# arneschneuing/DiffSBDD

Hardware: AMD Instinct MI355X
Metric: sampled ligands/sec (500-step DDPM, fullatom_cond) at 1/2/4/8 MI355X (higher is better)
Workload: dtype f32

## Files before the change

diffsbdd_amd/_lib.py:

```python
from __future__ import annotations

import ctypes as C
import os

_HERE = os.path.dirname(os.path.abspath(__file__))
LIB_PATH = os.environ.get("DSBDD_LIB") or os.path.join(_HERE, "libdiffsbdd_hip.so")
ABI_VERSION = 6

OK, ERR_ARG, ERR_STATE, ERR_CAPACITY, ERR_LAUNCH = 0, -1, -2, -3, -4
STATUS_NAN, STATUS_EDGE_OVERFLOW = 1, 2
MOL_MAX_ATOMS, MOL_STATS, FP_WORDS = 128, 8, 64

G_NAMES = ["ATOM_ENC_W0T", "ATOM_ENC_B0", "ATOM_ENC_W1T", "ATOM_ENC_B1",
           "RES_ENC_W0T", "RES_ENC_B0", "RES_ENC_W1T", "RES_ENC_B1",
           "ATOM_DEC_W0T", "ATOM_DEC_B0", "ATOM_DEC_W1T", "ATOM_DEC_B1",
           "RES_DEC_W0T", "RES_DEC_B0", "RES_DEC_W1T", "RES_DEC_B1",
           "EMB_WT", "EMB_B", "EMBOUT_WT", "EMBOUT_B"]
GCL_NAMES = ["E1_WT", "E1_WD", "E1_WD0", "E1_TAB", "E2_WT", "E2_B", "ATT_W", "ATT_B",
             "N1_WT", "N1_B", "N2_WT", "N2_B"]
EQ_NAMES = ["C1_WT", "C_WD", "C_WD0", "C_TAB", "C_W2T", "C_B2",
            "X_WD", "X_WD0", "X_TAB", "X_W2T", "X_B2", "W3"]
OPT_PRUNE, OPT_CONE, OPT_GRANULE16, OPT_EMU, OPT_SPLITK, OPT_SHELL, OPT_TAIL = 0, 1, 2, 3, 4, 5, 6
(BUF_EDGE_ROW, BUF_EDGE_COL, BUF_EDGE_D0, BUF_ROW_PTR, BUF_H, BUF_X, BUF_NODE_BATCH, BUF_DEG,
 BUF_LEVEL, BUF_LEVEL_LIST, BUF_LEVEL_COUNT, BUF_LEVEL_END, BUF_LROW_PTR, BUF_LEDGE_ROW, BUF_LEDGE_COL,
# ... 32 lines not shown
                ("gd0", C.c_void_p)]


class OptimCfg(C.Structure):
    _fields_ = [(n, C.c_double) for n in ("lr", "beta1", "beta2", "eps", "weight_decay")] + [("clip_grad", C.c_int32)]


_P = C.c_void_p
_I64 = C.c_int64
_I32 = C.c_int32
_F = C.c_float

SIGNATURES = {
    "dsbdd_abi_version": (C.c_int, []),
    "dsbdd_last_error": (C.c_char_p, []),
    "dsbdd_engine_create": (C.c_int, [C.POINTER(Config), C.POINTER(_P)]),
    "dsbdd_engine_destroy": (None, [_P]),
    "dsbdd_engine_weight_slots": (C.c_int, [_P]),
    "dsbdd_engine_set_weights": (C.c_int, [_P, C.POINTER(_P), C.c_int]),
    "dsbdd_engine_workspace_bytes": (C.c_size_t, [_P, _I64, _I64, _I64, _I64]),
    "dsbdd_engine_bind_workspace": (C.c_int, [_P, _P, C.c_size_t, _I64, _I64, _I64, _I64]),
    "dsbdd_engine_set_trace": (C.c_int, [_P, _P, _P]),
    "dsbdd_engine_set_pocket_frame": (C.c_int, [_P, _P, _P, _P, _P, _P, _I64, _I64, _I64, _I64, _I64, _I64]),
    "dsbdd_engine_clear_pocket_frame": (C.c_int, [_P]),
    "dsbdd_dynamics_forward": (C.c_int, [_P, _P, _P, _P, _P, _I64, _P, _P, _I64, _I64, _I64,
                                         _P, _P, _I64, _P, _P, _P]),
    "dsbdd_engine_buffer": (C.c_int, [_P, C.c_int, C.POINTER(_P)]),
    "dsbdd_engine_shell_read": (C.c_int, [_P, C.c_int, C.c_int, _P, C.c_int64]),
    "dsbdd_engine_list2_read": (C.c_int, [_P, C.c_int, _P, C.c_int64]),
    "dsbdd_engine_graph_stats": (C.c_int, [_P, C.POINTER(_I64), C.POINTER(_I64), C.POINTER(_I64)]),
    "dsbdd_engine_last_plan": (C.c_int, [_P, C.POINTER(C.c_int32), C.POINTER(C.c_int32), C.c_int32,
                                         C.POINTER(C.c_int32), C.POINTER(C.c_int32)]),
    "dsbdd_engine_set_option": (C.c_int, [_P, C.c_int, C.c_int]),
    "dsbdd_engine_get_option": (C.c_int, [_P, C.c_int]),
    "dsbdd_engine_profile": (C.c_int, [_P, C.c_int, C.c_int]),
    "dsbdd_engine_profile_read": (C.c_int, [_P, C.POINTER(C.c_double), C.POINTER(_I64)]),
    "dsbdd_cond_reverse_update": (C.c_int, [_P, _P, _P, _P, _P, _P, _P, _I64, _I64, _I64,
                                            _I32, _I32, _F, _F, _F, _I32]),
    "dsbdd_joint_reverse_update": (C.c_int, [_P, _P, _P, _P, _P, _P, _P, _P, _P, _I64, _I64, _I64,
                                             _I32, _I32, _F, _F, _F, _I32]),
    "dsbdd_segment_mean3": (C.c_int, [_P, _P, _I32, _P, _I64, _I64, _P]),
    "dsbdd_cond_affine_noise": (C.c_int, [_P, _P, _P, _P, _P, _P, _I64, _I64, _I64, _I32, _I32, _F, _F, _I32]),
    "dsbdd_joint_affine_noise": (C.c_int, [_P, _P, _P, _P, _P, _P, _P, _I64, _I64, _I64, _I32, _I32, _F, _F,
                                           _I32, _I32]),
    "dsbdd_cond_repaint_update": (C.c_int, [_P, _P, _P, _P, _P, _P, _P, _P, _P, _P, _P, _I64, _I64, _I64,
                                            _I32, _I32, _F, _F, _F, _F, _I32, _I32]),
    "dsbdd_joint_repaint_update": (C.c_int, [_P] * 15 + [_I64, _I64, _I64, _I32, _I32, _F, _F, _F, _F, _I32]),
    "dsbdd_cond_step_keyed": (C.c_int, [_P] * 10 + [_I64, _I64, _I64, _I32, _I32, _F, _F, _F, _I32, _F, _F, _F, _I32,
                                        C.c_uint64, C.c_uint64, _I64, _P, _P, _F]),
    "dsbdd_randn_keyed": (C.c_int, [_P, _P, _P, _I64, _I32, _I64, _I64, _P, C.c_uint64, C.c_uint64,
                                    C.c_uint32]),
    "dsbdd_node_linear": (C.c_int, [_P, _P, _I32, _I32, _P, _I32, _I32, _P, _I32, _P, _P, _I32,
                                    _P, _I32, _I64, _I32, _I32]),
    "dsbdd_chain_split_host": (_I64, [_I32, _I32, _I32, _P, _P, _P, _I32, _I32, _P, _P, _I64]),
    "dsbdd_chain_split_probe": (C.c_int, [_P, _I32, _P, _I32, _I32, _P, _P, _P, _I32, _I32, _P, _P, _I64, _P]),
    "dsbdd_build_edges": (C.c_int, [_P, _P, _P, _P, _I64, _I64, _I64, C.POINTER(Config),
                                    _P, _P, _P, _P, _P, _P, _P, _P, _I64, _P]),
    "dsbdd_bond_orders": (C.c_int, [_P, _P, _P, _P, _I64, _I32, _P, _P, _P, C.c_float, C.c_float,
                                    C.c_float, _I32, _P]),
    "dsbdd_mol_graph_stats": (C.c_int, [_P, _P, _P, _P, _I64, _I32, _P, _I32, _I32, _P, _P, _P, _P, _P, _P]),
    "dsbdd_fp_diversity": (C.c_int, [_P, _P, _P, _I64, _P, _P]),
    "dsbdd_pose_check": (C.c_int, [_P, _P, _P, _P, _I64, _P, _P, _P, _P, _I64, _F, _F, _P, _P]),
    "dsbdd_vina_type": (C.c_int, [_P, _P, _P, _P, _I64, _I32, _P, _I32, _P, _P]),
    "dsbdd_vina_score": (C.c_int, [_P, _P, _P, _P, _I64, _P, _P, _P, _P, _P, _I64, _P, _P, _P]),
    "dsbdd_pack_ligands": (C.c_int, [_P, _P, _P, _P, _I32, _I64, _P, _P, _P, _I64, _I64, _I32, _P, _P, _P, _P, _P]),
    "dsbdd_train_scratch_bytes": (C.c_size_t, [_I32, _I64, _I64]),
    "dsbdd_train_wgrad_scratch_bytes": (C.c_size_t, [_I64, _I64, _I64]),
    "dsbdd_train_wgrad_plan_bytes": (C.c_size_t, [_I64, _I64, _I64]),
    "dsbdd_train_edge_rev": (C.c_int, [_P, _P, _P]),
    "dsbdd_train_sample_mean": (C.c_int, [_P, _P, _P, _P]),
    "dsbdd_train_gcl_forward": (C.c_int, [_P, _I32, _P, _P, _P, _F, _P, _P, C.c_size_t]),
    "dsbdd_train_gcl_backward": (C.c_int, [_P, _I32, _P, _P, _P, _F, _P, _P, _P, _P, C.c_size_t]),
    "dsbdd_train_coord_forward": (C.c_int, [_P, _I32, _P, _P, _I32, _P, _P, _I64, _F, _F, _I32, _F, _P, _P,
                                            C.c_size_t]),
    "dsbdd_train_coord_backward": (C.c_int, [_P, _I32, _P, _P, _I32, _P, _P, _I64, _I64, _F, _F, _I32, _F, _P, _P, _P,
                                             _P, _P, C.c_size_t]),
    "dsbdd_train_radial_backward": (C.c_int, [_P, _P, _P, _P, _P]),
    "dsbdd_train_wgrad": (C.c_int, [_P, _P, _I32, _P, _I32, _I64, _I32, _I32, _P, _P, C.c_size_t]),
    "dsbdd_train_colsum": (C.c_int, [_P, _P, _I32, _I64, _I32, _P, _P, C.c_size_t]),
    "dsbdd_train_net_create": (C.c_int, [C.POINTER(Config), C.POINTER(_P)]),
    "dsbdd_train_net_destroy": (None, [_P]),
    "dsbdd_train_net_param_count": (C.c_int, [_P]),
    "dsbdd_train_net_pack_bytes": (C.c_size_t, [_P]),
    "dsbdd_train_net_workspace_bytes": (C.c_size_t, [_P, C.POINTER(TrainGraph)]),
    "dsbdd_train_net_forward": (C.c_int, [_P, _P, C.POINTER(TrainGraph), C.POINTER(_P), _P, C.c_size_t, _P, C.c_size_t, _P, _P,
                                          _P, _I64, _I32, _P, _P, _P]),
    "dsbdd_train_net_backward": (C.c_int, [_P, _P, C.POINTER(TrainGraph), C.POINTER(_P), C.POINTER(_P), _P, C.c_size_t, _P,
                                           C.c_size_t, _I64, _P, _P, _P, _P]),
    "dsbdd_train_net_forward_held": (C.c_int, [_P, _P, C.POINTER(TrainGraph), C.POINTER(_P), _P, C.c_size_t, _P, C.c_size_t,
                                               _P, _P, _P, _I64, _I32, _P, _P, _P, _I32]),
    "dsbdd_train_net_backward_acc": (C.c_int, [_P, _P, C.POINTER(TrainGraph), C.POINTER(_P), C.POINTER(_P), _P, _P, C.c_size_t,
                                               _P, C.c_size_t, _I64, _P, _P, _P, _P]),
    "dsbdd_edge_capacity": (C.c_int, [_P, _P, _I64, _P, _I64, _I64, _P]),
    "dsbdd_loss_rows": (C.c_int, []),
    "dsbdd_loss_out_rows": (C.c_int, []),
    "dsbdd_loss_cond_pre": (C.c_int, [_P, C.POINTER(LossCfg)] + [_P] * 17),
    "dsbdd_loss_cond_post": (C.c_int, [_P, C.POINTER(LossCfg)] + [_P] * 8),
    "dsbdd_loss_cond_post_backward": (C.c_int, [_P, C.POINTER(LossCfg)] + [_P] * 9),
    "dsbdd_loss_joint_out_rows": (C.c_int, []),
    "dsbdd_loss_joint_pre": (C.c_int, [_P, C.POINTER(LossCfg)] + [_P] * 20),
    "dsbdd_loss_joint_post": (C.c_int, [_P, C.POINTER(LossCfg)] + [_P] * 10),
    "dsbdd_loss_joint_post_backward": (C.c_int, [_P, C.POINTER(LossCfg)] + [_P] * 14),
    "dsbdd_score_rows": (C.c_int, [_I32]),
    "dsbdd_score_cond_pre": (C.c_int, [_P, C.POINTER(LossCfg), _I32, _I64, _I64, _I64, _I64] + [_P] * 17),
    "dsbdd_score_cond_post": (C.c_int, [_P, C.POINTER(LossCfg), _I32, _I64, _I64, _I64, _I64] + [_P] * 7),
    "dsbdd_score_reduce": (C.c_int, [_P, _I64, _I32, _P, _P, _P, _P]),
# ... 60 lines not shown
```

diffsbdd_amd/csrc/capi_kernels.h:

```cpp
#pragma once

extern "C" {

int dsbdd_cond_reverse_update(void* stream, float* z_lig, float* xh_pocket, const float* eps_lig,
                              const float* noise, const int64_t* mask_lig, const int64_t* mask_pocket,
                              int64_t n_lig, int64_t n_pocket, int64_t batch, int32_t atom_nf,
                              int32_t residue_nf, float alpha_ts, float c_eps, float sigma, int32_t remove_com) {
  StreamDevice stream_device_(stream);
  if (!z_lig || !xh_pocket || !eps_lig || !noise || !mask_lig || !mask_pocket || batch < 1)
    return fail(DSBDD_ERR_ARG, "bad argument");
  hipLaunchKernelGGL(cond_update_kernel, dim3((int)batch), dim3(kThreads), 0, static_cast<hipStream_t>(stream),
                     z_lig, xh_pocket, eps_lig, noise, mask_lig, (int)n_lig, mask_pocket, (int)n_pocket,
                     3 + atom_nf, 3 + residue_nf, alpha_ts, c_eps, sigma, remove_com);
  HIP_TRY(hipGetLastError());
  return DSBDD_OK;
}

int dsbdd_joint_reverse_update(void* stream, float* z_lig, float* z_pocket, const float* eps_lig,
                               const float* eps_pocket, const float* noise_lig, const float* noise_pocket,
                               const int64_t* mask_lig, const int64_t* mask_pocket, int64_t n_lig,
                               int64_t n_pocket, int64_t batch, int32_t atom_nf, int32_t residue_nf,
                               float alpha_ts, float c_eps, float sigma, int32_t center_noise) {
  StreamDevice stream_device_(stream);
  if (!z_lig || !z_pocket || !eps_lig || !eps_pocket || !noise_lig || !noise_pocket || !mask_lig ||
// ... 81 lines not shown
  a.eps = eps_lig; a.u_alpha_ts = alpha_ts; a.u_c_eps = c_eps; a.u_sigma = sigma; a.repaint = repaint;
  a.seed = seed; a.draw = draw_index; a.sample_offset = sample_offset; a.sample_ids = sample_ids;
  a.t_word = t_word; a.t_next = t_next;
  hipLaunchKernelGGL(cond_step_keyed_kernel, dim3((int)batch), dim3(kThreads), 0, static_cast<hipStream_t>(stream), a);
  HIP_TRY(hipGetLastError());
  return DSBDD_OK;
}

int dsbdd_joint_repaint_update(void* stream, float* z_lig, float* z_pocket, float* scratch_lig,
                               float* scratch_pocket, const float* xh0_lig, const float* xh0_pocket,
                               const float* fixed_lig, const float* fixed_pocket, const float* noise_known_lig,
                               const float* noise_known_pocket, const float* noise_jump_lig,
                               const float* noise_jump_pocket, const int64_t* mask_lig,
                               const int64_t* mask_pocket, int64_t n_lig, int64_t n_pocket, int64_t batch,
                               int32_t atom_nf, int32_t residue_nf, float alpha_s, float sigma_s,
                               float alpha_ts, float sigma_ts, int32_t jump) {
  StreamDevice stream_device_(stream);
  if (!z_lig || !z_pocket || !scratch_lig || !scratch_pocket || !xh0_lig || !xh0_pocket || !fixed_lig ||
      !fixed_pocket || !noise_known_lig || !noise_known_pocket || (jump && (!noise_jump_lig || !noise_jump_pocket)) ||
      !mask_lig || !mask_pocket || batch < 1)
    return fail(DSBDD_ERR_ARG, "bad argument");
  JointRepaintArgs a{z_lig, z_pocket, scratch_lig, scratch_pocket, xh0_lig, xh0_pocket, fixed_lig, fixed_pocket,
                     noise_known_lig, noise_known_pocket, noise_jump_lig, noise_jump_pocket, mask_lig, mask_pocket,
                     (int)n_lig, (int)n_pocket, 3 + atom_nf, 3 + residue_nf, alpha_s, sigma_s, alpha_ts, sigma_ts,
                     jump};
  hipLaunchKernelGGL(joint_repaint_kernel, dim3((int)batch), dim3(kThreads), 0, static_cast<hipStream_t>(stream), a);
  HIP_TRY(hipGetLastError());
  return DSBDD_OK;
}

int dsbdd_randn_keyed(void* stream, float* out, const int64_t* mask, int64_t n_rows, int32_t n_cols,
                      int64_t batch, int64_t sample_offset, const int64_t* sample_ids, uint64_t seed,
                      uint64_t draw_index, uint32_t stream_id) {
  StreamDevice stream_device_(stream);
  (void)batch;
  if (!out || !mask || n_rows < 0 || n_cols < 1) return fail(DSBDD_ERR_ARG, "bad argument");
  const int64_t n = n_rows * n_cols;
  if (n == 0) return DSBDD_OK;
  hipLaunchKernelGGL(randn_keyed_kernel, dim3((int)((n + 255) / 256)), dim3(256), 0,
                     static_cast<hipStream_t>(stream), out, mask, (int)n_rows, (int)n_cols, sample_offset,
                     sample_ids, seed, draw_index, stream_id);
  HIP_TRY(hipGetLastError());
  return DSBDD_OK;
}

int dsbdd_node_linear(void* stream, const float* A1, int32_t lda1, int32_t K1, const float* A2, int32_t lda2,
                      int32_t K2, const float* WT, int32_t ldw, const float* bias, const float* R, int32_t ldr,
                      float* C, int32_t ldc, int64_t M, int32_t N, int32_t act) {
  StreamDevice stream_device_(stream);
  if (!A1 || !WT || !C || K1 < 1 || K2 < 0 || (K2 > 0 && !A2) || (ldw & 3) || N > ldw ||
      (reinterpret_cast<uintptr_t>(WT) & 15))
    return fail(DSBDD_ERR_ARG, "bad argument (WT must be 16-byte aligned with ldw % 4 == 0)");
  HIP_TRY(nl(static_cast<hipStream_t>(stream), A1, lda1, K1, A2, lda2, K2, WT, ldw, bias, R, ldr, C, ldc, M, N, act));
  return DSBDD_OK;
}

static bool chain_split_args_ok(int32_t M, int32_t n_proj, const void* proj_N, const void* proj_first, const void* proj_count,
                                int32_t H, int32_t grid, const void* header, const void* pieces, int64_t capacity) {
  return header && capacity >= 0 && (capacity == 0 || pieces) && grid >= 1 && (H == 64 || H == 128 || H == 192 || H == 256) &&
         n_proj >= 0 && n_proj <= kChainMaxProj && (n_proj == 0 || (proj_N && proj_first && proj_count)) && M <= (8 << 20);
}
static const char* const kChainSplitBadArg =
    "bad argument (null output, grid < 1, H not 64 / 128 / 192 / 256, more than 3 projections or more than 8 M rows)";

int64_t dsbdd_chain_split_host(int32_t M, int32_t do_mlp, int32_t n_proj, const int32_t* proj_N,
                               const int32_t* proj_first, const int32_t* proj_count, int32_t H, int32_t grid,
                               uint32_t* header, int32_t* pieces, int64_t capacity) {
  if (!chain_split_args_ok(M, n_proj, proj_N, proj_first, proj_count, H, grid, header, pieces, capacity))
    return fail(DSBDD_ERR_ARG, kChainSplitBadArg);
  ChainSplitIn in{};
  in.M = M; in.do_mlp = do_mlp; in.n_proj = n_proj; in.H = H; in.grid = grid;
  for (int q = 0; q < n_proj; ++q) { in.N[q] = proj_N[q]; in.first[q] = proj_first[q]; in.count[q] = proj_count[q]; }
  const ChainSplit sp(in);
  sp.report(header);
  return chain_split_list(sp, grid, grid, ~0u, pieces, capacity);
}

int dsbdd_chain_split_probe(void* stream, int32_t M, const int32_t* m_count, int32_t do_mlp, int32_t n_proj,
                            const int32_t* proj_N, const int32_t* proj_first, const int32_t* const* proj_count,
                            int32_t H, int32_t grid, uint32_t* header, int32_t* pieces, int64_t capacity,
                            int64_t* n_pieces) {
  StreamDevice stream_device_(stream);
  if (!n_pieces || !chain_split_args_ok(M, n_proj, proj_N, proj_first, proj_count, H, grid, header, pieces, capacity))
    return fail(DSBDD_ERR_ARG, kChainSplitBadArg);
  NodeChainArgs a{};
  a.M = M; a.m_count = m_count; a.do_mlp = do_mlp; a.n_proj = n_proj;
  for (int q = 0; q < n_proj; ++q) { a.proj[q].N = proj_N[q]; a.proj[q].first = proj_first[q]; a.proj[q].count = proj_count[q]; }
  hipLaunchKernelGGL(chain_split_probe_kernel, dim3(grid), dim3(64), 0, static_cast<hipStream_t>(stream), a, (int)H, header,
                     pieces, (long long)capacity, reinterpret_cast<long long*>(n_pieces));
  HIP_TRY(hipGetLastError());
  return DSBDD_OK;
}

int dsbdd_bond_orders(void* stream, const float* x, const int32_t* atom_type, const int32_t* mol_off,
                      int64_t batch, int32_t n_types, const float* bonds1, const float* bonds2,
                      const float* bonds3, float margin1, float margin2, float margin3, int32_t n_max,
                      int8_t* order) {
  StreamDevice stream_device_(stream);
  if (!x || !atom_type || !mol_off || !bonds1 || !bonds2 || !bonds3 || !order || batch < 1 || n_types < 1 ||
      n_max < 1)
    return fail(DSBDD_ERR_ARG, "bad argument");
  hipStream_t s = static_cast<hipStream_t>(stream);
  HIP_TRY(hipMemsetAsync(order, 0, (size_t)batch * n_max * n_max, s));
  BondArgs a{x, atom_type, mol_off, bonds1, bonds2, bonds3, margin1, margin2, margin3, n_types, n_max,
             reinterpret_cast<signed char*>(order)};
  hipLaunchKernelGGL(bond_orders_kernel, dim3((unsigned)batch), dim3(64), 0, s, a);
// ... 132 lines not shown
```

diffsbdd_amd/csrc/geometry.h:

```cpp
#pragma once
#include "common.h"
#include "graph_parts.h"
#include "radius_graph.h"

namespace dsbdd {

__global__ void prep_assemble_kernel(const int64_t* mask_lig, int n_lig, const int64_t* mask_poc, int n_poc, int B,
                                     int* node_batch, int* lig_off, int* poc_off, int* tile_ctr, const float* xh_lig,
                                     int dl, const float* xh_poc, int dp, const float* t, int t_count, float* x,
                                     float* x_in, float* h0, int J, int JP) {
  const int i = blockIdx.x * blockDim.x + threadIdx.x;
  prep_offsets(i, mask_lig, n_lig, mask_poc, n_poc, B, lig_off, poc_off, tile_ctr);
  if (i >= n_lig + n_poc) return;
  const int b = prep_node(i, mask_lig, n_lig, mask_poc, node_batch);
  const float* src = i < n_lig ? xh_lig + (size_t)i * dl : xh_poc + (size_t)(i - n_lig) * dp;
  const float a0 = src[0], a1 = src[1], a2 = src[2];
  x[3 * i] = a0; x[3 * i + 1] = a1; x[3 * i + 2] = a2;
  x_in[3 * i] = a0; x_in[3 * i + 1] = a1; x_in[3 * i + 2] = a2;
  h0[(size_t)i * JP + J] = t[t_count == 1 ? 0 : b];
  for (int k = J + 1; k < JP; ++k) h0[(size_t)i * JP + k] = 0.f;
}

__global__ __launch_bounds__(kThreads) void sample_mean_kernel(const float* x, const int* lig_off,
                                                               const int* poc_off, int n_lig,
                                                               float* mean) {
  __shared__ float red[3][kThreads];
  sample_mean_body(x, lig_off, poc_off, n_lig, mean, red);
}

struct CoordSums {
  const float* xagg; const float* xhead; int n_q;
  size_t xagg_stride, xhead_stride;
  const int* row_ptr; const int* deg;
  int max_tile, shift;
};

__device__ __forceinline__ void coord_row_update(float* x, const CoordSums& p, int k) {
  const int i = k / 3, c = k - 3 * i;
  const int d = p.deg[i];
  if (d == 0) return;
  const int s = p.row_ptr[i], t0 = s >> p.shift, t1 = min((s + d - 1) >> p.shift, p.max_tile);
  float tot = 0.f;
  for (int q = 0; q < p.n_q; ++q) {
    float a = p.xagg[q * p.xagg_stride + k];
    for (int T = t0 + 1; T <= t1; ++T) a += p.xhead[q * p.xhead_stride + 4 * (size_t)T + c];
    tot += a;
  }
  x[k] += tot;
}

__global__ void coord_update_kernel(float* x, CoordSums p, int n_upd3) {
  const int idx = blockIdx.x * blockDim.x + threadIdx.x;
  if (idx < n_upd3) coord_row_update(x, p, idx);
}

__global__ __launch_bounds__(kThreads) void coord_update_mean_kernel(float* x, CoordSums p, int n_upd,
                                                                     const int* lig_off, const int* poc_off,
                                                                     int n_lig, float* mean) {
  __shared__ float red[3][kThreads];
  const SampleRows r = sample_rows(lig_off, poc_off, n_lig, blockIdx.x);
  for (int seg = 0; seg < 2; ++seg) {
    const int a = seg ? r.p0 : r.l0, e = min(seg ? r.p1 : r.l1, n_upd);
    for (int k = 3 * a + (int)threadIdx.x; k < 3 * e; k += kThreads) coord_row_update(x, p, k);
  }
  if (!mean) return;
// ... 41 lines not shown
```

diffsbdd_amd/csrc/level_list.h:

```cpp
#pragma once
#include "common.h"
#include "graph_parts.h"

namespace dsbdd {

struct LevelArgs {
  const int* node_batch; const int* lig_off; const int* poc_off; int n_lig; int B;
  int* lvl;
  const int* deg;
  const int* row_ptr_nat;
  const int* erow_nat; const int* ecol_nat; const float* ed0_nat;
  int* seg_rows;
  int* seg_edges;
  int* node_base;
  int* edge_base;
  int* lvl_cnt;
  int* lvl_end;
  int* lvl_list;
  int* row_ptr;
  int* erow; int* ecol; float* ed0; int e_cap;
  unsigned long long* stats;
  int node_off; int edge_off;
  int e_cap_nat;
  const float* mean_x; float* mean_out;
  int n_shell;
  int* sh_seg;
  int* sh_deg; int* sh_ptr;
  int* sh_row; int* sh_col; float* sh_d0; int sh_cap;
  int* sh_cnt;
  unsigned long long* sh_stats;
};

constexpr int kLvlRows = 2048;
constexpr int kLvlEdges = 8192;

__device__ __forceinline__ void levels_rows_global(const LevelArgs& a, const SampleRows& r, int* s_rows, int* s_edges,
                                                   int* s_shell) {
  const int t = threadIdx.x;
  for (int k = 2; k < kLevels - 1; ++k) {
    __syncthreads();
    for (int i = r.p0 + t; i < r.p1; i += kThreads) {
      if (a.lvl[i] != kLevels - 1) continue;
      const int s = a.row_ptr_nat[i], d = a.deg[i];
      bool hit = false;
      for (int e = max(s, 0); e < min(s + d, a.e_cap_nat) && !hit; ++e) {
        const int j = a.ecol_nat[e];
        hit = j >= a.n_lig && a.lvl[j] == k - 1;
      }
      if (hit) a.lvl[i] = k;
    }
  }
  __syncthreads();
  for (int i = r.p0 + t; i < r.p1; i += kThreads) {
    const int L = a.lvl[i];
    atomicAdd(&s_rows[L], 1);
    atomicAdd(&s_edges[L], a.deg[i]);
    if (L >= 2 && L - 2 < a.n_shell) {
      const int s = a.row_ptr_nat[i], d = a.deg[i];
      int d2 = 0;
      for (int e = max(s, 0); e < min(s + d, a.e_cap_nat); ++e) {
        const int j = a.ecol_nat[e];
        d2 += (j < a.n_lig || a.lvl[j] < L) ? 1 : 0;
      }
      a.sh_deg[i] = d2;
      atomicAdd(&s_shell[L - 2], d2);
    }
  }
}

constexpr int kLvlPer = kLvlEdges / kThreads;
constexpr int kLvlBatch = 8;
constexpr int kLvlStage = 16;
constexpr int kLvlLig = 0xffff;
static_assert(kLvlPer % kLvlBatch == 0 && kLvlPer % kLvlStage == 0 && kLvlRows < kLvlLig, "codes: row << 16 | column");

__device__ __forceinline__ void levels_stage(const LevelArgs& a, const SampleRows& r, int e0, int ne, int (&code)[kLvlPer],
                                             int* s_lvl, int* s_deg, int* s_cnt) {
  const int t = threadIdx.x, np = r.p1 - r.p0;
  for (int i = t; i < np; i += kThreads) { s_lvl[i] = a.lvl[r.p0 + i]; s_deg[i] = a.deg[r.p0 + i]; s_cnt[i] = 0; }
#pragma unroll
  for (int u = 0; u < kLvlPer; ++u) code[u] = -1;
  if (ne <= 0) return;
#pragma unroll
  for (int g = 0; g < kLvlPer; g += kLvlStage) {
    if (g * kThreads >= ne) break;
    int row[kLvlStage], col[kLvlStage];
#pragma unroll
// ... 132 lines not shown
    const int cn = t == kLevels - 1 ? a.node_off + carry_n : a.node_base[(t + 1) * a.B];
    const int ce = t == kLevels - 1 ? a.edge_off + carry_e : a.edge_base[(t + 1) * a.B];
    unsigned long long ed = 0;
    if (a.stats) {
      int own = 0;
      for (int k = t * a.B; k < (t + 1) * a.B; ++k) own += a.seg_edges[k];
      s_wave[t] = own;
      __threadfence_block();
      __builtin_amdgcn_wave_barrier();
      for (int k = 0; k <= t; ++k) ed += (unsigned long long)s_wave[k];
    }
    level_end_write(a, t, cn, ce, ed);
  }
}

__device__ __forceinline__ void level_bases(const LevelArgs& a, int k, int lane, int& nb, int& eb) {
  int sn = 0, se = 0;
  for (int k0 = 0; k0 < k; k0 += 64) {
    const int kk = k0 + lane;
    if (kk < k) { sn += a.seg_rows[kk]; se += align_edges(a.seg_edges[kk]); }
  }
  nb = a.node_off + wave_sum_i(sn);
  eb = a.edge_off + wave_sum_i(se);
}

__global__ __launch_bounds__(kThreads) void level_place_kernel(LevelArgs a, int fold_scan = 0) {
  static_assert(kThreads / 64 >= kLevels - 1, "one wave per pocket level");
  const int b = blockIdx.x, lane = threadIdx.x & 63, w = threadIdx.x >> 6;
  if (fold_scan && b == 0 && w == kThreads / 64 - 1) {
    unsigned long long ed_run = 0;
    for (int t = 0; t < kLevels; ++t) {
      int cn, ce;
      level_bases(a, (t + 1) * a.B, lane, cn, ce);
      int own = 0;
      for (int k0 = t * a.B; k0 < (t + 1) * a.B; k0 += 64) { const int kk = k0 + lane; if (kk < (t + 1) * a.B) own += a.seg_edges[kk]; }
      ed_run += (unsigned long long)wave_sum_i(own);
      if (lane == 0) level_end_write(a, t, cn, ce, ed_run);
    }
  }
  if (w == 0) {
    const int l0 = a.lig_off[b], l1 = a.lig_off[b + 1];
    int nb, eb;
    if (fold_scan) level_bases(a, b, lane, nb, eb); else { nb = a.node_base[b]; eb = a.edge_base[b]; }
    const int s0 = l0 < l1 ? a.row_ptr_nat[l0] : 0;
    for (int i = l0 + lane; i < l1; i += 64) {
      a.lvl_list[nb + (i - l0)] = i;
      a.row_ptr[i] = eb + (a.row_ptr_nat[i] - s0);
    }
    pad_fill(eb + a.seg_edges[b], lane, a.erow, a.ecol, a.ed0, a.e_cap);
  }
  const int L = w + 1;
  if (L >= kLevels) return;
  const int p0 = a.n_lig + a.poc_off[b], p1 = a.n_lig + a.poc_off[b + 1];
  int n_run, e_run;
  if (fold_scan) level_bases(a, L * a.B + b, lane, n_run, e_run);
  else { n_run = a.node_base[L * a.B + b]; e_run = a.edge_base[L * a.B + b]; }
  const int sl = L - 2;
  const bool shell = sl >= 0 && sl < a.n_shell;
  int s_run = 0;
  if (shell) {
    int sp = 0;
    for (int k0 = 0; k0 < b; k0 += 64) {
      const int kk = k0 + lane;
      if (kk < b) sp += align_edges(a.sh_seg[sl * a.B + kk]);
    }
    s_run = wave_sum_i(sp);
  }
  const int s_begin = s_run;
  for (int i0 = p0; i0 < p1; i0 += 64) {
    const int i = i0 + lane;
    const bool mine = i < p1 && a.lvl[i] == L;
    const int d = mine ? a.deg[i] : 0;
    const unsigned long long m = __ballot(mine);
    const int incl = wave_scan_incl(d, lane);
    if (mine) {
      a.lvl_list[n_run + __popcll(m & ((1ull << lane) - 1ull))] = i;
      a.row_ptr[i] = e_run + incl - d;
    }
    n_run += __popcll(m);
    e_run += __shfl(incl, 63);
    if (shell) {
      const int d2 = mine ? a.sh_deg[i] : 0;
      const int incl2 = wave_scan_incl(d2, lane);
      if (mine) a.sh_ptr[i] = s_run + incl2 - d2;
      s_run += __shfl(incl2, 63);
    }
  }
  pad_fill(e_run, lane, a.erow, a.ecol, a.ed0, a.e_cap);
  if (shell) {
    const size_t o = (size_t)sl * a.sh_cap;
    const int to = pad_fill(s_run, lane, a.sh_row + o, a.sh_col + o, a.sh_d0 + o, a.sh_cap);
    if (lane == 0) {
      if (b == a.B - 1) a.sh_cnt[sl] = to;
      if (a.sh_stats) {
        const int own = s_run - s_begin;
        atomicAdd(&a.sh_stats[3 * sl], (unsigned long long)own);
        atomicAdd(&a.sh_stats[3 * sl + 1], (unsigned long long)(to - s_begin));
        atomicAdd(&a.sh_stats[3 * sl + 2], (unsigned long long)(a.seg_edges[L * a.B + b] - own));
        if (b == 0 && sl == 0) atomicAdd(&a.sh_stats[3 * kShellLists], 1ull);
      }
    }
  }
}

__global__ void level_copy_kernel(LevelArgs a, int n_nodes) {
  const int total = min(a.row_ptr_nat[n_nodes], a.e_cap_nat);
  for (int e = blockIdx.x * blockDim.x + threadIdx.x; e < total; e += gridDim.x * blockDim.x) {
    const int i = a.erow_nat[e];
    if (i < 0 || i >= n_nodes) continue;
    const int pos = a.row_ptr[i] + (e - a.row_ptr_nat[i]);
    if (pos >= 0 && pos < a.e_cap) { a.erow[pos] = i; a.ecol[pos] = a.ecol_nat[e]; a.ed0[pos] = a.ed0_nat[e]; }
    const int L = i >= a.n_lig ? a.lvl[i] : 0;
    if (L >= 2 && L - 2 < a.n_shell) {
      const int j = a.ecol_nat[e];
      if (j < a.n_lig || a.lvl[j] < L) {
        int rank = 0;
        for (int q = max(a.row_ptr_nat[i], 0); q < e; ++q) {
          const int jq = a.ecol_nat[q];
          rank += (jq < a.n_lig || a.lvl[jq] < L) ? 1 : 0;
        }
        const int ps = a.sh_ptr[i] + rank;
        const size_t o = (size_t)(L - 2) * a.sh_cap;
        if (ps >= 0 && ps < a.sh_cap) { a.sh_row[o + ps] = i; a.sh_col[o + ps] = j; a.sh_d0[o + ps] = a.ed0_nat[e]; }
      }
    }
  }
}

__global__ void ghost_setup_kernel(const int* erow3, const int* ecol3, const float* ed03, const int* row_ptr3,
                                   const int* deg3, int n3, int id_src, int id_dst, int* erow, int* ecol,
                                   float* ed0, int e_cap, int* deg, int* row_ptr, int* lvl_list,
                                   const float* xframe, float* x) {
  const int total = min(row_ptr3[n3], e_cap);
  for (int p = blockIdx.x * blockDim.x + threadIdx.x; p < total; p += gridDim.x * blockDim.x) {
    const int r = erow3[p];
    erow[p] = r < 0 ? -1 : r - id_src + id_dst;
    ecol[p] = r < 0 ? 0 : ecol3[p] - id_src + id_dst;
    ed0[p] = ed03[p];
  }
  for (int i = blockIdx.x * blockDim.x + threadIdx.x; i < n3; i += gridDim.x * blockDim.x) {
    deg[id_dst + i] = deg3[i];
    row_ptr[id_dst + i] = row_ptr3[i];
    lvl_list[i] = id_dst + i;
    x[3 * (id_dst + i)] = xframe[3 * i]; x[3 * (id_dst + i) + 1] = xframe[3 * i + 1];
    x[3 * (id_dst + i) + 2] = xframe[3 * i + 2];
  }
}

__global__ __launch_bounds__(kThreads) void gather_rows_kernel(float* dst, const float* src, const int* rows, int n,
                                                               int H) {
  const int i = (blockIdx.x * kThreads + threadIdx.x) >> 6, lane = threadIdx.x & 63;
  if (i >= n) return;
  const float* a = src + (size_t)rows[i] * H;
  float* b = dst + (size_t)i * H;
  for (int k = 4 * lane; k < H; k += 256) *reinterpret_cast<float4*>(b + k) = ld4(a + k);
}

__global__ __launch_bounds__(kThreads) void canon_fill_kernel(float* h, const int* lvl, const int* twin_local,
                                                              int n_lig, int n_nodes, int ghost_base, int lo,
                                                              int hi, int H, float* pq = nullptr, int ldpq = 0) {
  const int i = n_lig + ((blockIdx.x * kThreads + threadIdx.x) >> 6), lane = threadIdx.x & 63;
  if (i >= n_nodes) return;
  const int L = lvl[i];
  if (L <= lo || L > hi) return;
  const int g = ghost_base + twin_local[i - n_lig];
  const float* src = h + (size_t)g * H;
  float* dst = h + (size_t)i * H;
  for (int k = 4 * lane; k < H; k += 256) *reinterpret_cast<float4*>(dst + k) = ld4(src + k);
  if (pq)
    for (int k = 4 * lane; k < ldpq; k += 256)
      *reinterpret_cast<float4*>(pq + (size_t)i * ldpq + k) = ld4(pq + (size_t)g * ldpq + k);
}

}
```

diffsbdd_amd/csrc/node_linear.h:

```cpp
#pragma once
#include "common.h"

namespace dsbdd {

struct NodeLinearArgs {
  const float* A1; int lda1; int K1;
  const float* A2; int lda2; int K2;
  const float* WT; int ldw;
  const float* bias;
  const float* R; int ldr;
  float* C; int ldc;
  int M; int N; int act;
  const int* row_idx; const int* m_count;
};

template <int BM, bool VEC_A>
__global__ __launch_bounds__(kThreads) void node_linear_kernel(NodeLinearArgs p) {
  constexpr int BN = 128, BK = 32, LDA = BM + 1;
  constexpr int RT = BM / 64;
  constexpr int AI = BM / 32;
  __shared__ float sA[BK * LDA];
  __shared__ float sB[BK * BN];

  const int t = threadIdx.x, lane = t & 63, w = t >> 6;
// ... 194 lines not shown

  int ro[16];
#pragma unroll
  for (int r = 0; r < 16; ++r) {
    const int rl = m0 + w * 32 + mfma_row(r, lane);
    ro[r] = rl < M ? (p.row_idx ? p.row_idx[rl] : rl) : -1;
  }
#pragma unroll
  for (int c = 0; c < CT; ++c) {
    const int col = n0 + c * 32 + j;
    const float bv = p.bias ? p.bias[col] : 0.f;
    f32x16 res;
#pragma unroll
    for (int r = 0; r < 16; ++r) res[r] = (p.R && ro[r] >= 0) ? p.R[(size_t)ro[r] * p.ldr + col] : 0.f;
#pragma unroll
    for (int r = 0; r < 16; ++r) {
      if (ro[r] < 0) continue;
      float v = acc[c][r] + bv;
      if (p.act == 1) v = silu(v);
      p.C[(size_t)ro[r] * p.ldc + col] = v + res[r];
    }
  }
}


template <int CT>
__global__ __launch_bounds__(kThreads, (CT == 4 ? 3 : 4)) void node_gemm_kernel(NodeGroupArgs ga, int balance) {
  constexpr int BN = 32 * CT, BK = node_bk(CT);
  constexpr int LDSF = 2 * BK * BN > 2 * node_bk(CT > 1 ? CT / 2 : 1) * (BN / 2) ? 2 * BK * BN
                                                                                 : 2 * node_bk(CT > 1 ? CT / 2 : 1) * (BN / 2);
  __shared__ float sB[LDSF];
  const NodeLinearArgs& p = ga.p[blockIdx.z];
  const int M = p.m_count ? min(p.M, *p.m_count) : p.M;
  const int m_tiles = (M + 127) / 128, gy = p.N / BN;
  int n_full = m_tiles;
  if (CT > 1 && balance > 0) n_full = (m_tiles * gy / balance) * balance / gy;
  const int id = blockIdx.x;
  if (id < n_full * gy) {
    node_gemm_tile<CT>(p, (id / gy) * 128, (id % gy) * BN, M, sB);
  } else if (CT > 1) {
    const int id2 = id - n_full * gy, rt = n_full + id2 / (2 * gy);
    if (rt >= m_tiles) return;
    node_gemm_tile<(CT > 1 ? CT / 2 : 1)>(p, rt * 128, (id2 % (2 * gy)) * (BN / 2), M, sB);
  }
}

struct Mlp2Problem {
  const float* in; int ld_in; int K0;
  const float* W0T; int ldw0; const float* b0; int M1;
  const float* W1T; int ldw1; const float* b1; int n_out;
  float* out; int ld_out; int rows;
};
struct Mlp2Args { Mlp2Problem p[2]; };
constexpr int kMlp2Rows = 32, kMlp2MaxK = 128, kMlp2MaxMid = 40, kMlp2MaxOut = 128;

__global__ __launch_bounds__(kThreads) void mlp2_kernel(Mlp2Args a) {
  __shared__ float sW0[kMlp2MaxK * kMlp2MaxMid];
  __shared__ float sW1[kMlp2MaxMid * kMlp2MaxOut];
  __shared__ float sIn[kMlp2Rows * (kMlp2MaxK + 1)];
  __shared__ float sMid[kMlp2Rows * (kMlp2MaxMid + 1)];
  const Mlp2Problem& p = a.p[blockIdx.y];
  const int t = threadIdx.x, r0 = blockIdx.x * kMlp2Rows;
  if (r0 >= p.rows) return;
  const int nr = min(kMlp2Rows, p.rows - r0);
  for (int i = t; i < p.K0 * p.M1; i += kThreads) sW0[i] = p.W0T[(size_t)(i / p.M1) * p.ldw0 + i % p.M1];
  for (int i = t; i < p.M1 * p.n_out; i += kThreads) sW1[i] = p.W1T[(size_t)(i / p.n_out) * p.ldw1 + i % p.n_out];
  for (int i = t; i < nr * p.K0; i += kThreads)
    sIn[(i / p.K0) * (kMlp2MaxK + 1) + i % p.K0] = p.in[(size_t)(r0 + i / p.K0) * p.ld_in + i % p.K0];
  __syncthreads();
  for (int i = t; i < nr * p.M1; i += kThreads) {
    const int r = i / p.M1, j = i % p.M1;
    float v = p.b0[j];
    const float* x = sIn + r * (kMlp2MaxK + 1);
    for (int k = 0; k < p.K0; ++k) v = fmaf(x[k], sW0[k * p.M1 + j], v);
    sMid[r * (kMlp2MaxMid + 1) + j] = silu(v);
  }
  __syncthreads();
  for (int i = t; i < nr * p.n_out; i += kThreads) {
    const int r = i / p.n_out, c = i % p.n_out;
    float v = p.b1[c];
    const float* m = sMid + r * (kMlp2MaxMid + 1);
    for (int j = 0; j < p.M1; ++j) v = fmaf(m[j], sW1[j * p.n_out + c], v);
    p.out[(size_t)(r0 + r) * p.ld_out + c] = v;
  }
}

inline bool mlp2_fits(const Mlp2Problem& p) {
  return p.K0 <= kMlp2MaxK && p.M1 <= kMlp2MaxMid && p.n_out <= kMlp2MaxOut;
}

inline hipError_t launch_mlp2(hipStream_t s, const Mlp2Problem* p, int n) {
  Mlp2Args a{};
  int rows = 0;
  for (int i = 0; i < n; ++i) { a.p[i] = p[i]; rows = max(rows, p[i].rows); }
  if (rows <= 0) return hipSuccess;
  hipLaunchKernelGGL(mlp2_kernel, dim3((rows + kMlp2Rows - 1) / kMlp2Rows, n), dim3(kThreads), 0, s, a);
  return hipGetLastError();
}

inline bool aligned16(const void* p) { return (reinterpret_cast<uintptr_t>(p) & 15) == 0; }

inline bool vec_ok(const NodeLinearArgs& a) {
  return aligned16(a.A1) && (a.lda1 % 4 == 0) && (a.K1 % 4 == 0) &&
         (a.K2 == 0 || (aligned16(a.A2) && (a.lda2 % 4 == 0) && (a.K2 % 4 == 0)));
}

inline int gemm_ct(const NodeLinearArgs& a, int forced_ct, bool allow_small = true) {
// ... 82 lines not shown
```

include/diffsbdd_hip.h:

```cpp
#ifndef DIFFSBDD_HIP_H
#define DIFFSBDD_HIP_H

#include <stddef.h>
#include <stdint.h>

#ifdef __cplusplus
extern "C" {
#endif

#define DSBDD_ABI_VERSION 6

enum {
  DSBDD_OK = 0,
  DSBDD_ERR_ARG = -1,
  DSBDD_ERR_STATE = -2,
  DSBDD_ERR_CAPACITY = -3,
  DSBDD_ERR_LAUNCH = -4
};

enum {
  DSBDD_STATUS_NAN = 1,
  DSBDD_STATUS_EDGE_OVERFLOW = 2
};

// ... 110 lines not shown
int dsbdd_joint_reverse_update(void* stream, float* z_lig, float* z_pocket, const float* eps_lig,
                               const float* eps_pocket, const float* noise_lig,
                               const float* noise_pocket, const int64_t* mask_lig,
                               const int64_t* mask_pocket, int64_t n_lig, int64_t n_pocket,
                               int64_t batch, int32_t atom_nf, int32_t residue_nf, float alpha_ts,
                               float c_eps, float sigma, int32_t center_noise);

int dsbdd_segment_mean3(void* stream, const float* x, int32_t ld, const int64_t* mask, int64_t n_rows,
                        int64_t batch, float* out);

int dsbdd_cond_affine_noise(void* stream, float* z_lig, float* xh_pocket, const float* noise,
                            const int64_t* mask_lig, const int64_t* mask_pocket, int64_t n_lig,
                            int64_t n_pocket, int64_t batch, int32_t atom_nf, int32_t residue_nf, float a,
                            float sigma, int32_t remove_com);

int dsbdd_joint_affine_noise(void* stream, float* z_lig, float* z_pocket, const float* noise_lig,
                             const float* noise_pocket, const int64_t* mask_lig, const int64_t* mask_pocket,
                             int64_t n_lig, int64_t n_pocket, int64_t batch, int32_t atom_nf,
                             int32_t residue_nf, float a, float sigma, int32_t center_noise,
                             int32_t remove_com);

int dsbdd_cond_repaint_update(void* stream, float* z_lig, float* xh_pocket, float* scratch_lig,
                              const float* xh0_lig, const float* com_pocket0, const float* fixed,
                              const float* noise_known, const float* noise_resample, const int64_t* mask_lig,
                              const int64_t* mask_pocket, int64_t n_lig, int64_t n_pocket, int64_t batch,
                              int32_t atom_nf, int32_t residue_nf, float alpha_s, float sigma_s,
                              float alpha_ts, float sigma_ts, int32_t resample, int32_t remove_com);

int dsbdd_cond_step_keyed(void* stream, float* z_lig, float* xh_pocket, const float* eps_lig, float* scratch_lig,
                          const float* xh0_lig, const float* com_pocket0, const float* fixed, const int64_t* mask_lig,
                          const int64_t* mask_pocket, int64_t n_lig, int64_t n_pocket, int64_t batch, int32_t atom_nf,
                          int32_t residue_nf, float alpha_ts, float c_eps, float sigma, int32_t repaint, float alpha_s,
                          float sigma_s, float sigma_ts, int32_t remove_com, uint64_t seed, uint64_t draw_index,
                          int64_t sample_offset, const int64_t* sample_ids, float* t_word, float t_next);

int dsbdd_joint_repaint_update(void* stream, float* z_lig, float* z_pocket, float* scratch_lig,
                               float* scratch_pocket, const float* xh0_lig, const float* xh0_pocket,
                               const float* fixed_lig, const float* fixed_pocket, const float* noise_known_lig,
                               const float* noise_known_pocket, const float* noise_jump_lig,
                               const float* noise_jump_pocket, const int64_t* mask_lig,
                               const int64_t* mask_pocket, int64_t n_lig, int64_t n_pocket, int64_t batch,
                               int32_t atom_nf, int32_t residue_nf, float alpha_s, float sigma_s,
                               float alpha_ts, float sigma_ts, int32_t jump);

int dsbdd_randn_keyed(void* stream, float* out, const int64_t* mask, int64_t n_rows,
                      int32_t n_cols, int64_t batch, int64_t sample_offset,
                      const int64_t* sample_ids, uint64_t seed, uint64_t draw_index,
                      uint32_t stream_id);

int dsbdd_node_linear(void* stream, const float* A1, int32_t lda1, int32_t K1, const float* A2,
                      int32_t lda2, int32_t K2, const float* WT, int32_t ldw, const float* bias,
                      const float* R, int32_t ldr, float* C, int32_t ldc, int64_t M, int32_t N,
                      int32_t act);

int64_t dsbdd_chain_split_host(int32_t M, int32_t do_mlp, int32_t n_proj, const int32_t* proj_N,
                               const int32_t* proj_first, const int32_t* proj_count, int32_t H, int32_t grid,
                               uint32_t* header, int32_t* pieces, int64_t capacity);

int dsbdd_chain_split_probe(void* stream, int32_t M, const int32_t* m_count, int32_t do_mlp, int32_t n_proj,
                            const int32_t* proj_N, const int32_t* proj_first, const int32_t* const* proj_count,
                            int32_t H, int32_t grid, uint32_t* header, int32_t* pieces, int64_t capacity,
                            int64_t* n_pieces);

int dsbdd_build_edges(void* stream, const float* x, const int64_t* mask_lig,
                      const int64_t* mask_pocket, int64_t n_lig, int64_t n_pocket, int64_t batch,
                      const dsbdd_config* cfg, int32_t* node_batch, int32_t* lig_off,
                      int32_t* poc_off, int32_t* deg, int32_t* row_ptr, int32_t* edge_row,
                      int32_t* edge_col, float* edge_d0, int64_t edge_capacity, int32_t* status);

typedef struct dsbdd_train_graph {
  const int32_t *erow, *ecol; const float* ed0;
  const int32_t *row_ptr, *deg;
  const int32_t* rev;
  const int32_t *node_batch, *lig_off, *poc_off;
  int64_t n_lig, n_nodes, n_edges, batch;
} dsbdd_train_graph;

typedef struct dsbdd_train_mlp {
  const float *P, *Q; int32_t ldpq;
  const float *wd, *wd0, *tab;
  const float *W2, *W2T, *b2;
  const float *head, *head_b;
} dsbdd_train_mlp;

typedef struct dsbdd_train_mlp_grad {
  float *dP, *dQ; int32_t ldo;
  float* d_vec;
  float* d_W2;
  float* gd0;
} dsbdd_train_mlp_grad;

size_t dsbdd_train_scratch_bytes(int32_t H, int64_t n_nodes, int64_t n_edges);
size_t dsbdd_train_wgrad_scratch_bytes(int64_t K, int64_t M, int64_t N);
size_t dsbdd_train_wgrad_plan_bytes(int64_t K, int64_t M, int64_t N);
int dsbdd_train_edge_rev(void* stream, const dsbdd_train_graph* g, int32_t* rev);
int dsbdd_train_sample_mean(void* stream, const float* x, const dsbdd_train_graph* g, float* mean);

int dsbdd_train_gcl_forward(void* stream, int32_t H, const dsbdd_train_graph* g, const dsbdd_train_mlp* m,
                            const float* x, float norm_factor, float* agg, void* scratch, size_t scratch_bytes);
int dsbdd_train_gcl_backward(void* stream, int32_t H, const dsbdd_train_graph* g, const dsbdd_train_mlp* m,
                             const float* x, float norm_factor, const float* d_agg,
                             const dsbdd_train_mlp_grad* out, float* d_x, void* scratch, size_t scratch_bytes);

int dsbdd_train_coord_forward(void* stream, int32_t H, const dsbdd_train_graph* g, const dsbdd_train_mlp* m,
                              int32_t n_mlp, const float* x, const float* mean, int64_t n_upd, float norm_constant,
                              float coords_range, int32_t use_tanh, float norm_factor, float* x_out, void* scratch,
// ... 158 lines not shown
```

Baseline: 42.38.

## Wave-parallelize level placement, shell ranking, and offsets; shrink mlp2 row tile

In level_copy_kernel, the per-thread serial loop that ranks shell edges is replaced by whole-wave ballot and popcount counting, and all loads are issued unconditionally with clamped indices. The placement kernel preloads level, degree and shell-degree values into registers for up to 8 trips before running the scans. Batch offsets in prep are now found with a wave-cooperative lower_bound. The mlp2 row tile drops from 32 to 8 rows, giving more blocks with less shared-memory input per block. Two new C API entry points (node_linear_rows, mlp2) are also exposed; they look like test or benchmark hooks.

```diff
diff --git a/diffsbdd_amd/_lib.py b/diffsbdd_amd/_lib.py
--- a/diffsbdd_amd/_lib.py
+++ b/diffsbdd_amd/_lib.py
@@ -108,6 +108,8 @@
                                     C.c_uint32]),
     "dsbdd_node_linear": (C.c_int, [_P, _P, _I32, _I32, _P, _I32, _I32, _P, _I32, _P, _P, _I32,
                                     _P, _I32, _I64, _I32, _I32]),
+    "dsbdd_node_linear_rows": (C.c_int, [_P, _P, _I32, _I32, _P, _I32, _P, _P, _I32, _I64, _I32, _I32, _P, _P, _I32]),
+    "dsbdd_mlp2": (C.c_int, [_P, _P, _I32, _I32, _P, _I32, _P, _I32, _P, _I32, _P, _I32, _P, _I32, _I64]),
     "dsbdd_chain_split_host": (_I64, [_I32, _I32, _I32, _P, _P, _P, _I32, _I32, _P, _P, _I64]),
     "dsbdd_chain_split_probe": (C.c_int, [_P, _I32, _P, _I32, _I32, _P, _P, _P, _I32, _I32, _P, _P, _I64, _P]),
     "dsbdd_build_edges": (C.c_int, [_P, _P, _P, _P, _I64, _I64, _I64, C.POINTER(Config),
diff --git a/diffsbdd_amd/csrc/capi_kernels.h b/diffsbdd_amd/csrc/capi_kernels.h
--- a/diffsbdd_amd/csrc/capi_kernels.h
+++ b/diffsbdd_amd/csrc/capi_kernels.h
@@ -157,6 +157,46 @@
       (reinterpret_cast<uintptr_t>(WT) & 15))
     return fail(DSBDD_ERR_ARG, "bad argument (WT must be 16-byte aligned with ldw % 4 == 0)");
   HIP_TRY(nl(static_cast<hipStream_t>(stream), A1, lda1, K1, A2, lda2, K2, WT, ldw, bias, R, ldr, C, ldc, M, N, act));
+  return DSBDD_OK;
+}
+
+int dsbdd_node_linear_rows(void* stream, const float* A1, int32_t lda1, int32_t K1, const float* WT, int32_t ldw,
+                           const float* bias, float* C, int32_t ldc, int64_t M, int32_t N, int32_t act,
+                           const int32_t* row_idx, const int32_t* m_count, int32_t kernel) {
+  StreamDevice stream_device_(stream);
+  if (!A1 || !WT || !C || K1 < 1 || M < 0 || M > 0x7fffffff || N < 1 || (ldw & 3) || N > ldw ||
+      (reinterpret_cast<uintptr_t>(WT) & 15) || (kernel != 1 && kernel != 2))
+    return fail(DSBDD_ERR_ARG, "bad argument (WT must be 16-byte aligned with ldw % 4 == 0; kernel is 1 or 2)");
+  if (M == 0) return DSBDD_OK;
+  hipStream_t s = static_cast<hipStream_t>(stream);
+  NodeLinearArgs a{A1, lda1, K1, nullptr, 0, 0, WT, ldw, bias, nullptr, 0, C, ldc, (int)M, N, act, row_idx, m_count};
+  if (kernel == 1) {
+    dim3 grid(((int)M + 63) / 64, (N + 127) / 128), block(kThreads);
+    if (vec_ok(a)) hipLaunchKernelGGL((node_linear_kernel<64, true>), grid, block, 0, s, a);
+    else           hipLaunchKernelGGL((node_linear_kernel<64, false>), grid, block, 0, s, a);
+  } else {
+    if (gemm_ct(a, 2) != 2) return fail(DSBDD_ERR_ARG, "the problem does not fit node_gemm_kernel<2>");
+    int balance = node_balance();
+    if (balance > 0 && (gemm_ct(a, 1) != 1 || balance % (N / 64) != 0)) balance = 0;
+    NodeGroupArgs ga{};
+    ga.p[0] = a;
+    const int gx = (((int)M + 127) / 128) * (N / 64) * (balance > 0 ? 2 : 1);
+    hipLaunchKernelGGL((node_gemm_kernel<2>), dim3(gx, 1, 1), dim3(kThreads), 0, s, ga, balance);
+  }
+  HIP_TRY(hipGetLastError());
+  return DSBDD_OK;
+}
+
+int dsbdd_mlp2(void* stream, const float* in, int32_t ld_in, int32_t K0, const float* W0T, int32_t ldw0, const float* b0,
+               int32_t M1, const float* W1T, int32_t ldw1, const float* b1, int32_t n_out, float* out, int32_t ld_out,
+               int64_t rows) {
+  StreamDevice stream_device_(stream);
+  if (!in || !W0T || !b0 || !W1T || !b1 || !out || rows < 0 || rows > 0x7fffffff || K0 < 1 || M1 < 1 || n_out < 1 ||
+      ld_in < K0 || ldw0 < M1 || ldw1 < n_out || ld_out < n_out)
+    return fail(DSBDD_ERR_ARG, "bad argument");
+  Mlp2Problem p{in, ld_in, K0, W0T, ldw0, b0, M1, W1T, ldw1, b1, n_out, out, ld_out, (int)rows};
+  if (!mlp2_fits(p)) return fail(DSBDD_ERR_ARG, "the widths do not fit mlp2_kernel");
+  HIP_TRY(launch_mlp2(static_cast<hipStream_t>(stream), &p, 1));
   return DSBDD_OK;
 }
 
diff --git a/diffsbdd_amd/csrc/geometry.h b/diffsbdd_amd/csrc/geometry.h
--- a/diffsbdd_amd/csrc/geometry.h
+++ b/diffsbdd_amd/csrc/geometry.h
@@ -10,7 +10,13 @@
                                      int dl, const float* xh_poc, int dp, const float* t, int t_count, float* x,
                                      float* x_in, float* h0, int J, int JP) {
   const int i = blockIdx.x * blockDim.x + threadIdx.x;
-  prep_offsets(i, mask_lig, n_lig, mask_poc, n_poc, B, lig_off, poc_off, tile_ctr);
+  if (tile_ctr && i < kTileCtrInts) tile_ctr[i] = 0;
+  const int lane = threadIdx.x & 63, n_waves = (gridDim.x * blockDim.x) >> 6;
+  for (int s = i >> 6; s < 2 * (B + 1); s += n_waves) {
+    const int v = s <= B ? s : s - (B + 1);
+    const int r = s <= B ? lower_bound_wave(mask_lig, n_lig, v, lane) : lower_bound_wave(mask_poc, n_poc, v, lane);
+    if (lane == 0) (s <= B ? lig_off : poc_off)[v] = r;
+  }
   if (i >= n_lig + n_poc) return;
   const int b = prep_node(i, mask_lig, n_lig, mask_poc, node_batch);
   const float* src = i < n_lig ? xh_lig + (size_t)i * dl : xh_poc + (size_t)(i - n_lig) * dp;
diff --git a/diffsbdd_amd/csrc/level_list.h b/diffsbdd_amd/csrc/level_list.h
--- a/diffsbdd_amd/csrc/level_list.h
+++ b/diffsbdd_amd/csrc/level_list.h
@@ -33,6 +33,7 @@
 
 constexpr int kLvlRows = 2048;
 constexpr int kLvlEdges = 8192;
+constexpr int kPlaceTrips = 8;
 
 __device__ __forceinline__ void levels_rows_global(const LevelArgs& a, const SampleRows& r, int* s_rows, int* s_edges,
                                                    int* s_shell) {
@@ -271,11 +272,25 @@
   const int L = w + 1;
   if (L >= kLevels) return;
   const int p0 = a.n_lig + a.poc_off[b], p1 = a.n_lig + a.poc_off[b + 1];
+  const int sl = L - 2;
+  const bool shell = sl >= 0 && sl < a.n_shell;
+  const int trips = (max(p1 - p0, 0) + 63) >> 6;
+  int t_lvl[kPlaceTrips], t_deg[kPlaceTrips], t_sdeg[kPlaceTrips];
+  if (trips <= kPlaceTrips) {
+#pragma unroll
+    for (int u = 0; u < kPlaceTrips; ++u) {
+      const int i = p0 + 64 * u + lane;
+      const bool in = i < p1;
+      const int is = in ? i : 0;
+      const int lv = a.lvl[is];
+      t_lvl[u] = in ? lv : -1;
+      t_deg[u] = a.deg[is];
+      t_sdeg[u] = shell ? a.sh_deg[is] : 0;
+    }
+  }
   int n_run, e_run;
   if (fold_scan) level_bases(a, L * a.B + b, lane, n_run, e_run);
   else { n_run = a.node_base[L * a.B + b]; e_run = a.edge_base[L * a.B + b]; }
-  const int sl = L - 2;
-  const bool shell = sl >= 0 && sl < a.n_shell;
   int s_run = 0;
   if (shell) {
     int sp = 0;
@@ -286,10 +301,7 @@
     s_run = wave_sum_i(sp);
   }
   const int s_begin = s_run;
-  for (int i0 = p0; i0 < p1; i0 += 64) {
-    const int i = i0 + lane;
-    const bool mine = i < p1 && a.lvl[i] == L;
-    const int d = mine ? a.deg[i] : 0;
+  auto place = [&](int i, bool mine, int d, int d2) {
     const unsigned long long m = __ballot(mine);
     const int incl = wave_scan_incl(d, lane);
     if (mine) {
@@ -299,10 +311,23 @@
     n_run += __popcll(m);
     e_run += __shfl(incl, 63);
     if (shell) {
-      const int d2 = mine ? a.sh_deg[i] : 0;
       const int incl2 = wave_scan_incl(d2, lane);
       if (mine) a.sh_ptr[i] = s_run + incl2 - d2;
       s_run += __shfl(incl2, 63);
+    }
+  };
+  if (trips <= kPlaceTrips) {
+#pragma unroll
+    for (int u = 0; u < kPlaceTrips; ++u) {
+      if (u >= trips) break;
+      const bool mine = t_lvl[u] == L;
+      place(p0 + 64 * u + lane, mine, mine ? t_deg[u] : 0, mine ? t_sdeg[u] : 0);
+    }
+  } else {
+    for (int i0 = p0; i0 < p1; i0 += 64) {
+      const int i = i0 + lane;
+      const bool mine = i < p1 && a.lvl[i] == L;
+      place(i, mine, mine ? a.deg[i] : 0, (mine && shell) ? a.sh_deg[i] : 0);
     }
   }
   pad_fill(e_run, lane, a.erow, a.ecol, a.ed0, a.e_cap);
@@ -324,24 +349,47 @@
 
 __global__ void level_copy_kernel(LevelArgs a, int n_nodes) {
   const int total = min(a.row_ptr_nat[n_nodes], a.e_cap_nat);
-  for (int e = blockIdx.x * blockDim.x + threadIdx.x; e < total; e += gridDim.x * blockDim.x) {
-    const int i = a.erow_nat[e];
-    if (i < 0 || i >= n_nodes) continue;
-    const int pos = a.row_ptr[i] + (e - a.row_ptr_nat[i]);
-    if (pos >= 0 && pos < a.e_cap) { a.erow[pos] = i; a.ecol[pos] = a.ecol_nat[e]; a.ed0[pos] = a.ed0_nat[e]; }
-    const int L = i >= a.n_lig ? a.lvl[i] : 0;
-    if (L >= 2 && L - 2 < a.n_shell) {
-      const int j = a.ecol_nat[e];
-      if (j < a.n_lig || a.lvl[j] < L) {
-        int rank = 0;
-        for (int q = max(a.row_ptr_nat[i], 0); q < e; ++q) {
+  const int lane = threadIdx.x & 63;
+  const unsigned long long below = (1ull << lane) - 1ull;
+  auto node = [&](int j) { return min(max(j, 0), n_nodes - 1); };
+  for (int ew = blockIdx.x * blockDim.x + (threadIdx.x & ~63); ew < total; ew += gridDim.x * blockDim.x) {
+    const int e = ew + lane, es = min(e, total - 1);
+    const int i = a.erow_nat[es], j = a.ecol_nat[es];
+    const float d0 = a.ed0_nat[es];
+    const bool row = e < total && i >= 0 && i < n_nodes;
+    const int is = node(i);
+    const int rp = a.row_ptr[is], rpn = a.row_ptr_nat[is], li = a.lvl[is], lj = a.lvl[node(j)];
+    const int sp = a.n_shell > 0 ? a.sh_ptr[is] : 0;
+    if (row) {
+      const int pos = rp + (e - rpn);
+      if (pos >= 0 && pos < a.e_cap) { a.erow[pos] = i; a.ecol[pos] = j; a.ed0[pos] = d0; }
+    }
+    if (a.n_shell <= 0) continue;
+    const int L = (row && i >= a.n_lig) ? li : 0;
+    const bool shell = L >= 2 && L - 2 < a.n_shell;
+    const bool low = shell && (j < a.n_lig || lj < L);
+    const unsigned long long m = __ballot(low);
+    if (m == 0) continue;
+    const int rs = max(rpn, 0);
+    const int rs0 = __shfl(rs, 0), L0 = __shfl(shell ? L : 0, 0);
+    int head = 0;
+    if (L0 >= 2) {
+      for (int q0 = rs0; q0 < ew; q0 += 64) {
+        const int q = q0 + lane;
+        bool lq = false;
+        if (q < ew) {
           const int jq = a.ecol_nat[q];
-          rank += (jq < a.n_lig || a.lvl[jq] < L) ? 1 : 0;
+          lq = jq < a.n_lig || a.lvl[node(jq)] < L0;
         }
-        const int ps = a.sh_ptr[i] + rank;
-        const size_t o = (size_t)(L - 2) * a.sh_cap;
-        if (ps >= 0 && ps < a.sh_cap) { a.sh_row[o + ps] = i; a.sh_col[o + ps] = j; a.sh_d0[o + ps] = a.ed0_nat[e]; }
-      }
+        head += __popcll(__ballot(lq));
+      }
+    }
+    if (low) {
+      const int first = max(rs, ew) - ew;
+      const int rank = __popcll(m & below & ~((1ull << first) - 1ull)) + (rs < ew ? head : 0);
+      const int ps = sp + rank;
+      const size_t o = (size_t)(L - 2) * a.sh_cap;
+      if (ps >= 0 && ps < a.sh_cap) { a.sh_row[o + ps] = i; a.sh_col[o + ps] = j; a.sh_d0[o + ps] = d0; }
     }
   }
 }
diff --git a/diffsbdd_amd/csrc/node_linear.h b/diffsbdd_amd/csrc/node_linear.h
--- a/diffsbdd_amd/csrc/node_linear.h
+++ b/diffsbdd_amd/csrc/node_linear.h
@@ -270,7 +270,7 @@
   float* out; int ld_out; int rows;
 };
 struct Mlp2Args { Mlp2Problem p[2]; };
-constexpr int kMlp2Rows = 32, kMlp2MaxK = 128, kMlp2MaxMid = 40, kMlp2MaxOut = 128;
+constexpr int kMlp2Rows = 8, kMlp2MaxK = 128, kMlp2MaxMid = 40, kMlp2MaxOut = 128;
 
 __global__ __launch_bounds__(kThreads) void mlp2_kernel(Mlp2Args a) {
   __shared__ float sW0[kMlp2MaxK * kMlp2MaxMid];
diff --git a/include/diffsbdd_hip.h b/include/diffsbdd_hip.h
--- a/include/diffsbdd_hip.h
+++ b/include/diffsbdd_hip.h
@@ -186,6 +186,14 @@
                       int32_t lda2, int32_t K2, const float* WT, int32_t ldw, const float* bias,
                       const float* R, int32_t ldr, float* C, int32_t ldc, int64_t M, int32_t N,
                       int32_t act);
+
+int dsbdd_node_linear_rows(void* stream, const float* A1, int32_t lda1, int32_t K1, const float* WT, int32_t ldw,
+                           const float* bias, float* C, int32_t ldc, int64_t M, int32_t N, int32_t act,
+                           const int32_t* row_idx, const int32_t* m_count, int32_t kernel);
+
+int dsbdd_mlp2(void* stream, const float* in, int32_t ld_in, int32_t K0, const float* W0T, int32_t ldw0,
+               const float* b0, int32_t M1, const float* W1T, int32_t ldw1, const float* b1, int32_t n_out,
+               float* out, int32_t ld_out, int64_t rows);
 
 int64_t dsbdd_chain_split_host(int32_t M, int32_t do_mlp, int32_t n_proj, const int32_t* proj_N,
                                const int32_t* proj_first, const int32_t* proj_count, int32_t H, int32_t grid,
```

Measured after the change: 42.58, median of 6. No clear change (+0.5%).
